# steve-the-bayesian/BOOM

Measured on AMD Instinct MI355X. Metric: Gibbs sweeps/sec (all chains), n=1e4 p=512 spike-slab, higher is better.
Workload: dtype f64; 1 GPU; BregVsSampler spike-and-slab n=1e4 p=512, 1024 chains per GPU, fp64 (BASELINE configs[1]); chains_per_gpu=1024, true_signals=16, burn_in=1000, parallelism=chains sharded, 1 GPU(s), suf_build=single device MFMA syrk

## Files before the change

boom_amd/capi.py:

```python
import ctypes as C
import os

import numpy as np

_HERE = os.path.dirname(os.path.abspath(__file__))
LIB_PATH = os.environ.get("BOOM_AMD_LIB", os.path.join(_HERE, "libboomamd.so"))

_dp = C.POINTER(C.c_double)
_u8p = C.POINTER(C.c_uint8)

SUMMARY_SCALARS = 16


class BoomAmdError(RuntimeError):

    def __init__(self, code, message):
        super().__init__(message)
        self.code = code


class BaConfig(C.Structure):
    _fields_ = [("device", C.c_int32), ("chains", C.c_int32),
                ("chain_offset", C.c_int64), ("seed", C.c_uint64),
                ("max_model_size_hint", C.c_int32), ("reserved", C.c_int32)]


_lib = None

SIGNATURES = {
    "ba_last_error": (C.c_char_p, []),
    "ba_engine_create": (C.c_int, [C.POINTER(BaConfig), C.POINTER(C.c_void_p)]),
    "ba_engine_destroy": (None, [C.c_void_p]),
    "ba_engine_info": (C.c_int, [C.c_void_p, C.POINTER(C.c_int32),
                                 C.POINTER(C.c_int32), C.POINTER(C.c_int32)]),
    "ba_build_suf_from_xy": (C.c_int, [C.c_void_p, C.c_int64, C.c_int32, _dp, _dp]),
    "ba_build_suf_from_xy_device": (C.c_int, [C.c_void_p, C.c_int64, C.c_int32,
                                              C.c_void_p, C.c_void_p]),
    "ba_suf_block_size": (C.c_size_t, [C.c_int32]),
    "ba_suf_partial_device": (C.c_int, [C.c_void_p, C.c_int64, C.c_int32, C.c_void_p,
                                        C.c_void_p, C.c_void_p]),
    "ba_set_suf_from_block_device": (C.c_int, [C.c_void_p, C.c_int64, C.c_int32, C.c_void_p]),
    "ba_upload_regression_suf": (C.c_int, [C.c_void_p, C.c_int32, _dp, _dp,
                                           C.c_double, C.c_double, C.c_double, _dp]),
    "ba_get_regression_suf": (C.c_int, [C.c_void_p, _dp, _dp, _dp, _dp, _dp, _dp]),
    "ba_set_slab": (C.c_int, [C.c_void_p, _dp, _dp]),
    "ba_set_spike": (C.c_int, [C.c_void_p, _dp, C.c_int64]),
    "ba_set_sigma_prior": (C.c_int, [C.c_void_p, C.c_double, C.c_double, C.c_double]),
    "ba_set_priors_ctor1": (C.c_int, [C.c_void_p, C.c_double, C.c_double,
                                      C.c_double, C.c_int32]),
    "ba_set_priors_ctor2": (C.c_int, [C.c_void_p, C.c_double, C.c_double,
                                      C.c_double, C.c_double, C.c_double, C.c_int32]),
    "ba_get_priors": (C.c_int, [C.c_void_p, _dp, _dp, _dp, _dp, _dp]),
    "ba_set_options": (C.c_int, [C.c_void_p, C.c_int32, C.c_double, C.c_int32, C.c_int32]),
    "ba_set_tuning": (C.c_int, [C.c_void_p, C.c_int32, C.c_int32, C.c_int32]),
    "ba_set_rebuild_policy": (C.c_int, [C.c_void_p, C.c_int32]),
    "ba_set_lookahead": (C.c_int, [C.c_void_p, C.c_int32]),
    "ba_draw_next": (C.c_int, [C.c_void_p]),
    "ba_set_state": (C.c_int, [C.c_void_p, C.c_int64, _u8p, _dp, C.c_double]),
    "ba_get_state": (C.c_int, [C.c_void_p, C.c_int64, _u8p, _dp, _dp]),
    "ba_get_states": (C.c_int, [C.c_void_p, _u8p, _dp, _dp]),
    "ba_logpri": (C.c_int, [C.c_void_p, C.c_int64, _dp]),
    "ba_seed": (C.c_int, [C.c_void_p, C.c_uint64]),
    "ba_sweep": (C.c_int, [C.c_void_p, C.c_int32]),
    "ba_sync": (C.c_int, [C.c_void_p]),
    "ba_log_model_prob": (C.c_int, [C.c_void_p, C.c_int32, _u8p, _dp]),
    "ba_set_sigsq": (C.c_int, [C.c_void_p, C.c_int64, C.c_double]),
    "ba_sss_set_slab": (C.c_int, [C.c_void_p, _dp, _dp, C.c_int32, C.c_int32]),
    "ba_sss_sweep": (C.c_int, [C.c_void_p, C.c_int32]),
    "ba_adaptive_set_options": (C.c_int, [C.c_void_p, C.c_int32, C.c_double, C.c_double]),
    "ba_adaptive_sweep": (C.c_int, [C.c_void_p, C.c_int32]),
    "ba_adaptive_get_rates": (C.c_int, [C.c_void_p, C.c_int64, _dp, _dp,
                                        C.POINTER(C.c_uint64)]),
    "ba_reset_summaries": (C.c_int, [C.c_void_p]),
    "ba_get_summaries": (C.c_int, [C.c_void_p, _dp, _dp, _dp, _dp]),
    "ba_summaries_device": (C.c_int, [C.c_void_p, C.c_void_p]),
    "ba_enable_traces": (C.c_int, [C.c_void_p, C.c_int32]),
    "ba_get_traces": (C.c_int, [C.c_void_p, C.c_int32, _dp, _dp, _dp]),
    "ba_enable_draws": (C.c_int, [C.c_void_p, C.c_int32]),
    "ba_get_draws": (C.c_int, [C.c_void_p, C.c_int64, C.c_int32, _u8p, _dp, _dp]),
    "ba_predict": (C.c_int, [C.c_void_p, C.c_int32, C.c_int32, C.c_int32, _dp, _dp]),
    "ba_get_coefficient_traces": (C.c_int, [C.c_void_p, C.c_int32, C.c_int32,
                                            C.POINTER(C.c_int32), _dp]),
    "ba_stream": (C.c_void_p, [C.c_void_p]),
    "ba_kernel_classes": (C.c_int32, []),
    "ba_kernel_class_name": (C.c_char_p, [C.c_int32]),
    "ba_set_kernel_timing": (C.c_int, [C.c_void_p, C.c_int32]),
    "ba_get_kernel_times": (C.c_int, [C.c_void_p, _dp, C.POINTER(C.c_int64), C.c_int32]),
    "ba_group_last_error": (C.c_char_p, []),
# ... 238 lines not shown

    def set_priors_ctor1(self, prior_nobs, expected_rsq, expected_model_size,
                         first_term_is_intercept=True):
        self._check(self.lib.ba_set_priors_ctor1(self._h, prior_nobs, expected_rsq,
                                                 expected_model_size,
                                                 int(first_term_is_intercept)))

    def set_priors_ctor2(self, prior_sigma_nobs, prior_sigma_guess, prior_beta_nobs,
                         diagonal_shrinkage, prior_inclusion_probability,
                         force_intercept=True):
        self._check(self.lib.ba_set_priors_ctor2(
            self._h, prior_sigma_nobs, prior_sigma_guess, prior_beta_nobs,
            diagonal_shrinkage, prior_inclusion_probability, int(force_intercept)))

    def get_priors(self):
        p = self.p
        b, om, pi = np.zeros(p), np.zeros(p * p), np.zeros(p)
        df, ss = C.c_double(), C.c_double()
        self._check(self.lib.ba_get_priors(self._h, _p(b), _p(om), _p(pi),
                                           C.byref(df), C.byref(ss)))
        return dict(b=b, ominv=om.reshape(p, p).T.copy(), pi=pi, df=df.value, ss=ss.value)

    def set_options(self, max_flips=-1, swap_threshold=0.8, draw_beta=True,
                    draw_sigma=True):
        self._check(self.lib.ba_set_options(self._h, max_flips, swap_threshold,
                                            int(draw_beta), int(draw_sigma)))

    def set_tuning(self, waves_per_chain=0, walk_policy=-1, kcap_start=0):
        self._check(self.lib.ba_set_tuning(self._h, waves_per_chain, walk_policy, kcap_start))

    def set_rebuild_policy(self, policy):
        self._check(self.lib.ba_set_rebuild_policy(self._h, int(policy)))

    def set_state(self, gamma, beta=None, sigsq=1.0, chain=-1):
        g = np.ascontiguousarray(gamma, dtype=np.uint8)
        bb = None if beta is None else _f64(beta)
        self._check(self.lib.ba_set_state(self._h, chain, _b(g), _p(bb), sigsq))

    def get_state(self, chain):
        p = self.p
        g = np.zeros(p, np.uint8)
        b = np.zeros(p)
        s = C.c_double()
        self._check(self.lib.ba_get_state(self._h, chain, _b(g), _p(b), C.byref(s)))
        return g, b, s.value

    def get_states(self):
        p, c = self.p, self.chains
        g = np.zeros((c, p), np.uint8)
        b = np.zeros((c, p))
        s = np.zeros(c)
        self._check(self.lib.ba_get_states(self._h, _b(g), _p(b), _p(s)))
        return g, b, s

    def seed(self, seed):
        self._check(self.lib.ba_seed(self._h, seed))

    def sweep(self, nsweeps=1, sync=True):
        self._check(self.lib.ba_sweep(self._h, nsweeps))
        if sync:
            self.sync()

    def sync(self):
        self._check(self.lib.ba_sync(self._h))

    def set_lookahead(self, n):
# ... 922 lines not shown
```

boom_amd/csrc/engine.hip:

```cpp
#include "engine_internal.h"

namespace boom_amd {

static thread_local std::string g_error = "";

int fail(int code, const std::string &msg) {
  g_error = msg;
  return code;
}

}

namespace {


const char *status_message(int st) {
  switch (st) {
    case CHAIN_NOT_PD:
      return "The posterior information matrix is not positive definite.  "
             "Check your data or consider adjusting your prior.";
    case CHAIN_NEGATIVE_SS:
      return "Illegal data caused negative sum of squares in "
             "Breg::set_reg_post_params.";
    case CHAIN_ILLEGAL_START:
// ... 289 lines not shown
  P.cm_idx = e->dcm_idx.ptr;
  P.cm_cor = e->dcm_cor.ptr;
  P.gamma = e->dgamma.ptr;
  P.beta = e->dbeta.ptr;
  P.sigsq = e->dsigsq.ptr;
  P.perm = e->dperm.ptr;
  P.rng_pos = e->dpos.ptr;
  P.status = e->dstatus.ptr;
  P.failures = e->dfail.ptr;
  P.todo = e->dtodo.ptr;
  P.maxk = e->dmaxk.ptr;
  P.trace_idx = e->dtrace_idx.ptr;
  P.model_scratch = e->dmodel.ptr;
  P.table_lp = e->dtab_lp.ptr;
  P.table_kind = e->dtab_kind.ptr;
  P.table_tag = e->dtab_tag.ptr;
  P.table_keep = e->table_ok ? 1 : 0;
  P.model_tag = e->dmodel_tag.ptr;
  P.model_keep = e->model_ok ? 1 : 0;
  P.suf_changed = (e->data_kind == DATA_STATE_SPACE || latent_data(e->data_kind)) ? 1 : 0;
  P.run_limit = 0;
  P.ran = nullptr;
  P.model_scratch_stride = (int64_t)ssvs_scalar_layout(64).total;
  P.big_kcap = e->big_kcap;
  P.big_model = e->dbig_model.ptr;
  P.big_model_stride = e->big_kcap > 0 ? (int64_t)ssvs_scalar_layout(e->big_kcap).total : 0;
  P.big_xs = e->dbig_xs.ptr;
  P.seed_lo = (uint32_t)e->seed;
  P.seed_hi = (uint32_t)(e->seed >> 32);
  P.stream = 0;
  P.mode = e->cur_mode;
  P.walk_policy = e->tune_walk_policy >= 0 ? e->tune_walk_policy : 1;
  P.rebuild_policy = e->tune_rebuild_policy;
  if (e->cur_mode == 1) {
    P.slab_scales = e->sss_slab_scales;
    P.stream = 3;
    P.rng_pos = e->dpos_sss.ptr;
    P.draw_sigma = 0;
    P.draw_beta = 1;
    P.cm_start = nullptr;
    P.max_flips = (e->sss_max_flips > 0) ? std::min(e->sss_max_flips, e->p) : e->p;
  }
  if (e->cur_mode == 1 && student_kind(e->data_kind) && !e->student_allow_selection)
    P.max_flips = 0;
  if (e->cur_mode == 1 && column_service(e->data_kind) && e->cols.V.count) {
    P.mode = (e->data_kind == DATA_LOGIT || e->data_kind == DATA_SS_LOGIT) ? 2 : 1;
    if (e->data_kind == DATA_MLOGIT) {
      P.mode = 3;
      P.flip_order = e->dml_order.ptr;
      P.wss = e->dml_wss.ptr;
      if (!e->mlogit_select) P.max_flips = 0;
    }
    P.V = e->cols.V.ptr;
    P.v_chain_stride = (int64_t)e->p * e->p;
    P.model_keep = 0;
    P.table_keep = 0;
    P.col_valid = e->cols.valid.ptr;
    P.col_words = e->cols.words;
    P.col_request = e->cols.wanted.ptr;
    P.v_diag = e->cols.vdiag.ptr;
  }
  if (e->cur_mode == 2) {
    P.mode = 0;
    P.stream = 4;
    P.rng_pos = e->dpos_ada.ptr;
    P.cm_start = nullptr;
// ... 864 lines not shown
  MUTATE(e);
  e->max_flips = max_flips;
  if (swap_threshold != e->swap_threshold) e->device_dirty = true;
  e->swap_threshold = swap_threshold;
  e->draw_beta = draw_beta;
  e->draw_sigma = draw_sigma;
  return BA_OK;
}

int ba_set_tuning(ba_engine *e, int32_t waves_per_chain, int32_t walk_policy,
                  int32_t kcap_start) {
  if (!e) return fail(BA_E_INVALID, "null engine");
  if (!(waves_per_chain == 0 || waves_per_chain == 1 || waves_per_chain == 2 || waves_per_chain == 4))
    return fail(BA_E_INVALID, "waves_per_chain must be 0, 1, 2 or 4");
  if (walk_policy < -1 || walk_policy > 4) return fail(BA_E_INVALID, "walk_policy must be in [-1, 4]");
  if (kcap_start < 0) return fail(BA_E_INVALID, "kcap_start must be non-negative");
  MUTATE(e);
  if (e->state_ready) {
    int rc = set_device(e);
    if (!rc) rc = ba_sync(e);
    if (rc) return rc;
  }
  e->tune_waves = waves_per_chain;
  e->tune_walk_policy = walk_policy;
  e->tune_kcap_start = kcap_start;
  e->device_dirty = true;
  return BA_OK;
}

int ba_set_rebuild_policy(ba_engine *e, int32_t policy) {
  if (!e) return fail(BA_E_INVALID, "null engine");
  if (policy != 0 && policy != 1) return fail(BA_E_INVALID, "rebuild_policy must be 0 or 1");
  e->tune_rebuild_policy = policy;
  return BA_OK;
}

int ba_set_slot_limit(ba_engine *e, int32_t uniforms) {
  if (!e) return fail(BA_E_INVALID, "null engine");
  if (uniforms < 0 || (uniforms & 1)) return fail(BA_E_INVALID, "uniforms must be even and non-negative");
  MUTATE(e);
  e->slot_limit = uniforms;
  return BA_OK;
}

int ba_set_state(ba_engine *e, int64_t chain, const uint8_t *gamma,
                 const double *beta, double sigsq) {
  ENGINE_PROLOGUE(e);
  if (e->p <= 0) return fail(BA_E_STATE, "set the regression data first");
  if (!gamma) return fail(BA_E_INVALID, "null argument");
  const int64_t C = e->cfg.chains;
  if (chain < -1 || chain >= C) return fail(BA_E_INVALID, "chain index out of range");
  if (latent_data(e->data_kind) && !student_kind(e->data_kind) && sigsq != 1.0)
    return fail(BA_E_INVALID, "the binomial samplers' latent data have unit variance: sigsq must be 1");
  if (chain < 0) la_discard(e);
  MUTATE(e);
  if (e->state_ready) {
    int rc = ba_sync(e);
    if (rc && chain >= 0) return rc;
    if (rc) {
      HIP_TRY(hipMemsetAsync(e->dstatus.ptr, 0, (size_t)C * 4, e->stream));
      HIP_TRY(hipMemsetAsync(e->dtodo.ptr, 0, (size_t)C * 4, e->stream));
    }
  }
  int rc = alloc_chain_state(e);
  if (rc) return rc;
  const size_t p = (size_t)e->p;
// ... 873 lines not shown
```

boom_amd/csrc/engine_internal.h:

```cpp
#pragma once
#include <hip/hip_runtime.h>

#include <algorithm>
#include <cmath>
#include <cstdio>
#include <cstdlib>
#include <cstring>
#include <limits>
#include <string>
#include <unordered_map>
#include <vector>

#include "../../include/boom_amd.h"
#include "kalman_params.h"
#include "ktimer.h"
#include "mlogit_params.h"
#include "probit_params.h"
#include "products.h"
#include "quantile_params.h"
#include "ss_filter_params.h"
#include "ssg_regholiday.h"
#include "ssg_spec.h"
#include "ssvs_params.h"
#include "student_params.h"
// ... 184 lines not shown
  DevBuf<int32_t> dran;
  bool table_ok = false;
  bool model_ok = false;
  int trace_stride = 0;
  DevBuf<double> dX, dy, dxtx, dxsum, dsufscal;

  int kcap = 0;
  int waves = 1;
  struct La {
    int len = 1, avail = 0, served = 0;
    struct Rows { std::vector<double> k, sig, beta; std::vector<uint16_t> idx; };
    std::unordered_map<int64_t, Rows> cache;
    bool synced = false;
    bool pipe = true;
    bool cur_piped = false;
    bool ahead = false;
    int slot = 0;
    hipEvent_t done[2] = {nullptr, nullptr};
    struct Snap {
      DevBuf<uint8_t> gamma;
      DevBuf<double> beta, sigsq, bsum, bsumsq, acc;
      DevBuf<uint16_t> perm;
      DevBuf<uint64_t> pos;
      DevBuf<int32_t> fail;
      DevBuf<uint32_t> inc;
    } snap;
  } la;
  int rec_cap = 64;
  bool big_active = false;
  int big_kcap = 0;
  DevBuf<double> dbig_model, dbig_xs;
  int tune_waves = 0, tune_walk_policy = -1, tune_kcap_start = 0;
  int tune_rebuild_policy = 0;
  int cur_mode = 0;
  int sss_slab_scales = 1;
  int sss_max_flips = -1;
  double v_scale = 1.0;
  double v_scale_want = 1.0;
  DevBuf<uint64_t> dpos_sss;
  uint64_t seed = 0;
  DevBuf<double> dada_birth, dada_death, dada_ws;
  DevBuf<uint64_t> dada_iter, dpos_ada;
  int ada_max_flips = 100;
  double ada_step = .001, ada_target = .345;

  bool ss_level_set = false, ss_initialized = false;
  int T = 0;
  DevBuf<double> dss_y, dss_X, dss_scratch;
  void *pinned = nullptr;
  size_t pinned_bytes = 0;
  uint64_t api_seq = 1, clean_seq = 0;
  int api_depth = 0;
  DevBuf<double> dss_yt, dss_Xt;
  DevBuf<uint32_t> dss_obs_mask;
  DevBuf<uint8_t> dss_obs;
  DevBuf<double> dxty_c, dyty_c, dnobs_c;
  DevBuf<double> dlev_sigsq, dlev_n, dlev_sumsq;
  DevBuf<uint64_t> dpos_level, dpos_state, dpos_forecast;
  hipStream_t stream2 = nullptr;
  hipEvent_t ev_state = nullptr, ev_prep[2] = {nullptr, nullptr};
  int ss_zbuf = 0;
  struct Pipe {
    hipStream_t stream = nullptr;
    hipEvent_t ev[4] = {}, join_ev = nullptr;
    DevBuf<int32_t> q, err;
    bool on = false;
// ... 250 lines not shown
```

boom_amd/csrc/ssvs_params.h:

```cpp
#pragma once
#include <stdint.h>

namespace boom_amd {

enum ChainStatus : int32_t {
  CHAIN_OK = 0,
  CHAIN_NOT_PD = 1,
  CHAIN_NEGATIVE_SS = 2,
  CHAIN_ILLEGAL_START = 3,
  CHAIN_RNG_BRANCH = 4,
  CHAIN_FORECAST_VARIANCE = 5,
  CHAIN_MODEL_TOO_LARGE = 6,
  CHAIN_NEED_COLUMN = 7,
  CHAIN_NEED_COLUMN_BIG = 8
};
enum { MLVS_ILLEGAL_START = 12 };

enum { SUMMARY_SCALARS = 16 };
enum {
  ACC_SWEEPS = 0,
  ACC_SIGSQ = 1,
  ACC_SIGSQ2 = 2,
  ACC_K = 3,
  ACC_ACCEPTS = 4,
// ... 76 lines not shown
  double *acc;
  double *trace_sigsq, *trace_logp, *trace_k;
  int32_t trace_stride;
  uint16_t *rec_idx;
  double *rec_beta;
  int32_t rec_cap;

  double *ada_birth, *ada_death;
  uint64_t *ada_iter;
  double ada_step, ada_target;
  int32_t ada_max_flips;
  int32_t *q_in, *q_out;
  int32_t *q_error;
  int32_t trace_row0;
  uint8_t *snap_gamma;
  double *snap_beta, *snap_sigsq, *snap_bsum, *snap_bsumsq, *snap_acc;
  uint16_t *snap_perm;
  uint64_t *snap_pos;
  int32_t *snap_fail;
  uint32_t *snap_inc;
  int32_t adaptive;
  double *ada_ws;

  int32_t big_kcap;
  double *big_model;
  int64_t big_model_stride;
  double *big_xs;
  const double *xty_planes;
  int32_t xty_nplanes;
  int64_t xty_plane_stride;
  const uint16_t *flip_order;
  const double *wss;
  int32_t rebuild_policy;
};

struct SsvsLds {
  uint32_t Lv, La, rdv, rda, w, bg, ctrl, park, g, perm0, perm1, oth, last, pred, gam, gam0, nbr, total;
};

static inline __host__ __device__ SsvsLds ssvs_lds_layout(int p, int kcap) {
  SsvsLds L;
  const uint32_t nb = (uint32_t)kcap / 8;
  const uint32_t fac = nb * (nb + 1) / 2 * 64 * 8;
  const uint32_t pv = ((((uint32_t)p + 1u) * 2) + 15u) & ~15u;
  uint32_t o = 0;
  L.Lv = o;    o += fac;
  L.La = o;    o += fac;
  L.rdv = o;   o += (uint32_t)kcap * 8;
  L.rda = o;   o += (uint32_t)kcap * 8;
  L.w = o;     o += (uint32_t)kcap * 8;
  L.bg = o;    o += (uint32_t)kcap * 8;
  L.ctrl = o;  o += 512;
  L.park = o;  o += 4 * 512;
  L.g = o;     o += (((uint32_t)kcap * 2) + 15u) & ~15u;
  L.perm0 = o; o += pv;
  L.perm1 = o; o += pv;
  L.oth = o;   o += pv;
  L.last = o;  o += 2 * pv;
  L.pred = o;  o += pv;
  L.gam = o;   o += ((uint32_t)p + 15u) & ~15u;
  L.gam0 = o;  o += ((uint32_t)p + 15u) & ~15u;
  L.nbr = o;   o += ((uint32_t)p + 15u) & ~15u;
  L.total = o;
  return L;
}

// ... 82 lines not shown
```

boom_amd/csrc/ssvs_sweep_body.h:

```cpp
#pragma once
#include "ssvs_device.h"

namespace boom_amd {

template <int NB, int W, int WPE, bool MLVS = false>
__device__ __forceinline__ void ssvs_sweep_body(SsvsParams P, int nsweeps, const int chain,
                                                unsigned char *smem) {
  constexpr bool SHUFFLE_MASKED = NB >= 6 && W > 1;
  P.V += (size_t)chain * (size_t)P.v_chain_stride;
  if (P.col_valid) {
    P.col_valid += (size_t)chain * (size_t)P.col_words;
    P.v_diag += (size_t)chain * (size_t)P.p;
  }
  int tid_ = threadIdx.x;
  BA_OPAQUE_V(tid_);
  int lane = tid_ & (WAVE - 1);
  const int wave = tid_ >> 6;
  const int p = P.p;
#ifdef BA_PSTAMPS
  long long pst[8];
  pst[0] = (long long)__builtin_readcyclecounter();
#endif
  constexpr int FOLD_Z = 16;
  const bool fold = (W == 1) && P.xty_planes != nullptr;
// ... 185 lines not shown
    if (j < p) {
      ch.gam[j] = (uint8_t)inc;
      ch.perm[j] = g_perm[j];
      ch.nbr[j] = (uint8_t)((P.cm_start != nullptr) && (P.cm_start[j + 1] > P.cm_start[j]));
    }
    const unsigned long long mask = __ballot(inc != 0);
    const int slot = k + __popcll(mask & ((1ull << lane) - 1ull));
    if (inc && slot < KCAP) ch.g[slot] = (uint16_t)j;
    k += __popcll(mask);
  }
  if (k > KCAP) status = CHAIN_MODEL_TOO_LARGE;
  ch.k = k;
  wave_sync();
  bool aborted = false;
  int need_col = -1;
  int kmax = k;
  int trace_at = (P.trace_row0 >= 0) ? P.trace_row0 : (P.trace_idx ? P.trace_idx[chain] : 0);

  uint64_t pos = uni((uint64_t)P.rng_pos[chain]);
  int failures = uni((int)P.failures[chain]);
  double sigsq = uni((double)P.sigsq[chain]);
  double beta_m = 0.0;
  int gprev = 0, kprev = 0;
  bool beta_valid = false;

  lds_f64 *sum_b = to_lds<double>(smem + lay.park + 512);
  lds_f64 *sum_b2 = to_lds<double>(smem + lay.park + 1024);
  AS_LDS int *sum_n = to_lds<int>(smem + lay.park + 1536);
  AS_LDS int *sum_g = to_lds<int>(smem + lay.park + 1792);
  sum_b[lane] = 0.0; sum_b2[lane] = 0.0; sum_n[lane] = 0; sum_g[lane] = -1;
  if (lane < 13) ctl[CT_ACC + lane] = (lane == ACC_MIN_MARGIN) ? BA_INF : 0.0;
  if (W == 2 && lane == 0) ((AS_LDS uint64_t *)(ctl + CT_NEXT))[0] = ~0ull;
  wave_sync();
#define ACC_ADD(slot, x) do { if (lane == 0) ctl[CT_ACC + (slot)] += (double)(x); } while (0)
#define ACC_MIN(x) do { if (lane == 0) ctl[CT_ACC + ACC_MIN_MARGIN] = fmin(ctl[CT_ACC + ACC_MIN_MARGIN], (x)); } while (0)
  int done = 0;

  const int nflips = P.max_flips;
  STAMP_DECL;
  StampCtx sx;
  sx.last = (long long)__builtin_readcyclecounter();
  for (int i = 0; i < 8; ++i) sx.ph[i] = 0.0;

  Model M;
  M.bad = 0; M.pd = true; M.logp = 0; M.lp = 0; M.ldv = 0; M.lda = 0; M.Q = 0; M.c = 0; M.SS = 0;
  Pending pe;
  pe.kind = EV_INIT; pe.f1 = pe.f2 = -1; pe.lu = 0; pe.lfw = pe.lrev = 0; pe.check_legal = false;
  enum { PH_BEGIN, PH_FLIPS, PH_SWAP, PH_TAIL, PH_JOIN, PH_COMMIT };
  int phase = PH_BEGIN, sweep = 0, i0 = 0;
  bool model_checked = false;
  int perm_sel = 0;
  bool use_table = false;
  int cur = 0, other_var = -1;
  bool other_ok = false, table_valid_other = false;
  const int model_tag_in = P.model_keep ? P.model_tag[chain] : 0;
  const bool model_kept = (model_tag_in & 0xff) == KCAP && status == CHAIN_OK;
  if (model_kept) cur = (model_tag_in >> 8) & 1;
  bind_slot(ch, P, chain, cur);
  bool table_valid = P.table_keep && model_kept && P.table_tag[chain] == model_tag_in;
  int fill_j = 0;
  bool spec = false;
  bool have_dr = false;
  int after_join = PH_COMMIT, spec_status = CHAIN_OK;
  bool commit_pending = false, gam0_fresh = false;
  lds_f64 *park = to_lds<double>(smem + lay.park);
  int stops_prev = table_valid ? 0 : (1 << 20), stops_now = 0;
  uint64_t flip_pos = 0, pos0 = pos;
  WinRng rng;
  rng.init(key, lane, pos);

  PSTAMP(3);
  if (model_kept) {
    {
      const SsvsScalarLayout S = ssvs_scalar_layout(KCAP);
      const double *sc = ch.sc_store + S.scal;
      const double s0 = sc[0], s1 = sc[1], s2 = sc[2], s3 = sc[3], s4 = sc[4], s5 = sc[5], s6 = sc[6], s7 = sc[7];
      restore_model<NB>(ch);
      M.logp = s0; M.lp = s1; M.ldv = s2; M.lda = s3;
      M.Q = s4; M.c = s5; M.SS = s6; M.pd = s7 != 0.0;
      unsigned long long u = (unsigned long long)ch.sc_store;
      asm volatile("s_dcache_inv\n\ts_waitcnt lgkmcnt(0)" : "+s"(u) : : "memory");
      ch.sc = (c_f64 *)u;
    }
    if (P.suf_changed) {
      refactor<true, MLVS>(P, ch, M, sx);
      if (M.bad) status = M.bad;
      else publish_model<NB>(ch, M);
    }
    if (lane == 0) {
      ctl[CT_LOGP] = M.logp; ctl[CT_LP] = M.lp; ctl[CT_LDV] = M.ldv;
      ctl[CT_LDA] = M.lda; ctl[CT_Q] = M.Q; ctl[CT_C] = M.c;
    }
    wave_sync();
    pe.kind = EV_NONE;
  }

  PSTAMP(4);
  while (status == CHAIN_OK) {
#ifdef BA_ROUND_KERNEL
    if constexpr ((W > 1 && !(NB == 4 && W == 2)) || (W == 1 && NB >= 4) || (MLVS && NB == 2)) {
#else
    constexpr bool PLAIN_211 = NB == 2 && W == 1;
    if constexpr ((W > 1 && !(NB == 4 && W == 2)) || (W == 1 && NB >= 4) || (MLVS && NB == 2) || PLAIN_211) {
#endif
      asm volatile("" : "+v"(lane));
      ch.lane = lane;
    }
    XCOUNT(sx, 6, 1);
    if (pe.kind != EV_NONE && !spec) {
      MSTAMP(sx, 7);
      XSTAMP(sx, 1);
      if (pe.kind == EV_FORCE && pe.f2 < 0 && other_ok && pe.f1 == other_var) {
        gam0_fresh = false;
        apply_flip(ch, pe.f1);
        cur ^= 1;
        bind_slot(ch, P, chain, cur);
        restore_model<NB>(ch);
        {
          const SsvsScalarLayout S = ssvs_scalar_layout(KCAP);
          const double *sc = ch.sc_store + S.scal;
          M.logp = sc[0]; M.lp = sc[1]; M.ldv = sc[2]; M.lda = sc[3];
          M.Q = sc[4]; M.c = sc[5]; M.SS = sc[6]; M.pd = sc[7] != 0.0;
          unsigned long long u = (unsigned long long)ch.sc_store;
          asm volatile("s_dcache_inv\n\ts_waitcnt lgkmcnt(0)" : "+s"(u) : : "memory");
          ch.sc = (c_f64 *)u;
        }
        if (lane == 0) {
          ctl[CT_LOGP] = M.logp; ctl[CT_LP] = M.lp; ctl[CT_LDV] = M.ldv;
          ctl[CT_LDA] = M.lda; ctl[CT_Q] = M.Q; ctl[CT_C] = M.c;
        }
        wave_sync();
        {
          const bool t = table_valid;
          table_valid = table_valid_other;
          table_valid_other = t;
        }
        ACC_ADD(ACC_ACCEPTS, 1);
#ifndef BA_STAMPS
        ACC_ADD(ACC_SLOT_HITS, 1);
#endif
// ... 132 lines not shown
            ctl[CT_ROLL + 0] = sigsq;
            ctl[CT_ROLL + 1] = (double)failures;
            ctl[CT_ROLL + 2] = beta_valid ? 1.0 : 0.0;
            ctl[CT_ROLL + 3] = 0.0;
          }
        }
        if (W > 1 && use_table && table_valid && model_checked && p > 1 && P.walk_policy != 3 && P.mode != 2 && !MLVS) {
          wave_sync();
          if (lane == 0) {
            ctl[CT_CMD] = (double)CMD_SHUFFLE_DECIDE;
            ctl[CT_I0] = 0.0;
            ctl[CT_NFLIPS] = (double)nflips;
            ctl[CT_PERMSEL] = (double)perm_sel;
            ctl[CT_CUR] = (double)cur;
            ((AS_LDS uint64_t *)(ctl + CT_POS))[0] = pos;
          }
          __syncthreads();
          fork_shuffle_targets<W>(key, pos, p, 0, lane, ch.oth);
          {
            lds_u16 *tmp = ch.perm;
            ch.perm = ch.perm_alt;
            ch.perm_alt = tmp;
            perm_sel ^= 1;
          }
          flip_pos = pos + (uint64_t)(p - 1);
          pos = flip_pos + (uint64_t)nflips;
          TSTAMP(sx, 2);
          XSTAMP(sx, 7);
          spec = true;
          spec_status = CHAIN_OK;
          i0 = 0;
          phase = commit_pending ? PH_COMMIT : PH_SWAP;
          STAMP(1);
          continue;
        }
        if constexpr (MLVS) {
          wave_sync();
          flip_pos = pos;
          pos = flip_pos + (uint64_t)nflips;
          if (!(M.logp > -BA_INF && M.logp < BA_INF)) { status = MLVS_ILLEGAL_START; aborted = true; }
        } else {
        if (W > 1) {
          if (lane == 0) {
            ctl[CT_CMD] = (double)CMD_UNIF;
            ((AS_LDS uint64_t *)(ctl + CT_POS))[0] = pos;
          }
          __syncthreads();
        }
        if (p > 1) shuffle_targets(key, pos, p, threadIdx.x, WAVE * W, ch.oth, P.mode == 2);
        if (W > 1) __syncthreads(); else wave_sync();
        STAMP(0);
        if (P.mode == 2) {
          if (lane == 0 && p > 1) {
            for (int i = 0; i < p; ++i) {
              const int j = ch.oth[i];
              const uint16_t a = ch.perm[i];
              ch.perm[i] = ch.perm[j];
              ch.perm[j] = a;
            }
          }
          wave_sync();
        } else if (p > 1) { parallel_shuffle<SHUFFLE_MASKED>(ch, sx); perm_sel ^= 1; }
        flip_pos = pos + (uint64_t)(P.mode == 2 ? p : (p > 0 ? p - 1 : 0));
        pos = flip_pos + (uint64_t)nflips;
        STAMP(1);
        if (!model_checked) {
          model_checked = true;
          if (!(M.logp > -BA_INF && M.logp < BA_INF)) {
            for (int j = 0; j < p; ++j) {
              const double pj = P.pi[j];
              const bool inc = ch.gam[j];
              if ((pj <= 0.0 && inc) || (pj >= 1.0 && !inc)) {
                if (!inc && ch.k >= KCAP) { status = CHAIN_MODEL_TOO_LARGE; aborted = true; break; }
                if (!inc && column_missing(P, j)) { status = CHAIN_NEED_COLUMN; need_col = j; aborted = true; break; }
                apply_flip(ch, j);
              }
            }
            pe.kind = EV_INIT;
            pe.check_legal = true;
          }
        }
        }
      }
      i0 = 0;
      phase = PH_FLIPS;
      XSTAMP(sx, 5);
      continue;
    }

    if (phase == PH_FLIPS) {
      XSTAMP(sx, 1);
      if (nflips == 0 || i0 >= nflips) {
        phase = PH_SWAP;
        XSTAMP(sx, 2);
        continue;
      }
      if (use_table && table_valid) {
        DecideResult dr;
        if (W > 1) {
          if (!have_dr) {
          MSTAMP(sx, 7);
          if (lane == 0) {
            ctl[CT_CMD] = (double)CMD_DECIDE;
            ctl[CT_I0] = (double)i0;
            ctl[CT_NFLIPS] = (double)nflips;
            ctl[CT_PERMSEL] = (double)perm_sel;
            ctl[CT_CUR] = (double)cur;
            ((AS_LDS uint64_t *)(ctl + CT_POS))[0] = flip_pos;
          }
          __syncthreads();
          if (P.walk_policy < 3 && P.mode != 2 && !MLVS) {
            spec = true;
            spec_status = CHAIN_OK;
            if (lane == 0) ctl[CT_ROLL + 3] = 1.0;
            MCOUNT(sx, 5, 1);
#ifndef BA_STAMPS
            ACC_ADD(ACC_REFORKS, 1);
#endif
            phase = commit_pending ? PH_COMMIT : PH_SWAP;
            XSTAMP(sx, 2);
            continue;
          }
          XSTAMP(sx, 2);
          __syncthreads();
          MSTAMP(sx, 0);
          XSTAMP(sx, 7);
          }
          have_dr = false;
          const lds_f64 *sl = ctl + CT_SLOT0 + CT_SLOT_STRIDE * 1;
// ... 102 lines not shown
      const int jf = uni((int)sl[SL_J]);
      const int kind = uni((int)sl[SL_KIND]);
      const int nprop = spos + 1 - i0;
      ACC_ADD(ACC_PROPOSALS, nprop);
      MCOUNT(sx, 4, stops_now == 0);
      ++stops_now;
      if (kind == STOP_BAD) {
        status = CHAIN_NEGATIVE_SS;
        break;
      }
      if (!ch.gam[jf] && ch.k >= KCAP) {
        status = CHAIN_MODEL_TOO_LARGE;
        aborted = true;
        break;
      }
      if (!ch.gam[jf] && column_missing(P, jf)) {
        status = CHAIN_NEED_COLUMN;
        need_col = jf;
        aborted = true;
        break;
      }
      pe.f1 = jf;
      if (kind == STOP_ACCEPT) {
        pe.kind = EV_FORCE;
      } else {
        pe.kind = EV_TRY_GE;
        pe.lu = uni((double)sl[SL_LOGU]);
      }
      i0 += nprop;
      XSTAMP(sx, 3);
      continue;
    }

    if (phase == PH_SWAP) {
      TSTAMP(sx, 7);
      XSTAMP(sx, 1);
      rng.set_pos(pos);
      if (nflips > 0) propose_swap(P, ch, rng, pe, &status);
      pos = rng.get_pos();
      phase = PH_TAIL;
      if (spec && (pe.kind != EV_NONE || status != CHAIN_OK)) {
        spec_status = status;
        status = CHAIN_OK;
        after_join = PH_TAIL;
        phase = PH_JOIN;
      }
      STAMP(4);
      TSTAMP(sx, 3);
      XSTAMP(sx, 7);
      continue;
    }

    if (phase == PH_JOIN) {
      MSTAMP(sx, 7);
      XSTAMP(sx, 1);
      __syncthreads();
      MSTAMP(sx, 1);
      XSTAMP(sx, 7);
      spec = false;
      i0 = uni((int)ctl[CT_I0]);
      const lds_f64 *sl = ctl + CT_SLOT0 + CT_SLOT_STRIDE * 1;
      if ((int)sl[SL_F] < 0) {
        ACC_MIN(sl[SL_MARGIN]);
        ACC_ADD(ACC_PROPOSALS, nflips - i0);
        status = spec_status;
        phase = after_join;
        if (after_join == PH_COMMIT && status == CHAIN_OK) {
          commit_pending = true;
          phase = PH_BEGIN;
        }
      } else {
        pos = flip_pos + (uint64_t)nflips;
        beta_m = park[lane];
        sigsq = ctl[CT_ROLL + 0];
        failures = (int)ctl[CT_ROLL + 1];
        beta_valid = ctl[CT_ROLL + 2] != 0.0;
        pe.kind = EV_NONE; pe.f1 = pe.f2 = -1; pe.lfw = pe.lrev = 0.0; pe.check_legal = false;
        have_dr = true;
        phase = PH_FLIPS;
        MCOUNT(sx, 6, ctl[CT_ROLL + 3]);
#ifndef BA_STAMPS
        ACC_ADD(ACC_REFORK_ROLLBACKS, ctl[CT_ROLL + 3]);
#endif
      }
      STAMP(3);
      XSTAMP(sx, 0);
      continue;
    }

    if (phase == PH_COMMIT) {
      TSTAMP(sx, 7);
      XSTAMP(sx, 1);
      k = ch.k;
      gprev = (lane < k) ? (int)ch.g[lane] : 0;
      kprev = k;
      kmax = k > kmax ? k : kmax;
      {
        const int gnow = (lane < k) ? gprev : -1;
        const int gold = sum_g[lane];
        if (__any(gnow != gold)) {
          const int n_old = sum_n[lane];
          if (gold >= 0 && n_old) {
            const size_t o = (size_t)chain * p + gold;
            const unsigned c0 = P.inc_count[o];
            const double b0 = P.beta_sum[o], q0 = P.beta_sumsq[o];
            P.inc_count[o] = c0 + (unsigned)n_old;
            P.beta_sum[o] = b0 + sum_b[lane];
            P.beta_sumsq[o] = q0 + sum_b2[lane];
          }
          sum_g[lane] = gnow; sum_n[lane] = 0; sum_b[lane] = 0.0; sum_b2[lane] = 0.0;
        }
        if (lane < k) {
          sum_n[lane] += 1;
          if (beta_valid) { sum_b[lane] += beta_m; sum_b2[lane] += beta_m * beta_m; }
        }
      }
      ACC_ADD(ACC_SIGSQ, sigsq);
      ACC_ADD(ACC_SIGSQ2, sigsq * sigsq);
      ACC_ADD(ACC_K, k);
      if (P.trace_sigsq && trace_at + sweep < P.trace_stride) {
        const size_t o = (size_t)chain * P.trace_stride + trace_at + sweep;
        if (lane == 0) {
          P.trace_sigsq[o] = sigsq;
          P.trace_logp[o] = M.logp;
          P.trace_k[o] = (double)k;
        }
        if (P.rec_idx && lane < k) {
          P.rec_idx[o * P.rec_cap + lane] = (uint16_t)gprev;
          P.rec_beta[o * P.rec_cap + lane] = beta_valid ? beta_m : 0.0;
        }
      }
      ++done;
      ++sweep;
      commit_pending = false;
      phase = spec ? PH_SWAP : PH_BEGIN;
      TSTAMP(sx, 0);
      XSTAMP(sx, 7);
      continue;
    }

    TSTAMP(sx, 7);
    XSTAMP(sx, 1);
    k = ch.k;
    rng.set_pos(pos);
    if (P.draw_sigma) {
      int bad = 0;
      const double DF = (k == 0) ? ch.DF : ((ch.DF - P.prior_df) + P.prior_df);
      const double SS = (k == 0) ? ch.ss0q : ((M.SS - P.prior_ss) + P.prior_ss);
      sigsq = uni(d_draw_variance(rng, DF, SS, P.sigma_max, &bad));
      if (bad) {
        if (!spec) { status = CHAIN_RNG_BRANCH; break; }
        spec_status = CHAIN_RNG_BRANCH; after_join = PH_COMMIT; phase = PH_JOIN;
        continue;
      }
    }
    pos = uni(rng.get_pos());
    STAMP(5);
    TSTAMP(sx, 4);
    if (P.draw_beta && k > 0) {
      if (!M.pd) {
        ++failures;
        if (!spec) { status = CHAIN_NOT_PD; break; }
        spec_status = CHAIN_NOT_PD; after_join = PH_COMMIT; phase = PH_JOIN;
        continue;
      }
      failures = 0;
      const double z = draw_normals(rng, k);
      pos = uni(rng.get_pos());
      TSTAMP(sx, 5);
      const double sigma = P.mode ? 1.0 : sqrt(sigsq);
      double y = (lane < k) ? ch.w[lane] + sigma * z : 0.0;
      const double rdm = (lane < k) ? ch.rdv[lane] : 0.0;
#pragma nounroll
      for (int ib = (k - 1) >> 3; ib >= 0; --ib) {
        double lr[8];
        const int base = bidx(ib * 8, lane < ib * 8 + 8 ? lane : 0);
#pragma unroll
        for (int t = 0; t < 8; ++t) lr[t] = ch.Lv[base + t * 8];
#pragma unroll
        for (int t = 7; t >= 0; --t) {
          const int i = ib * 8 + t;
          if (i < k) {
            const double xi = bcast_u(y * rdm, i);
            if (lane == i) y = xi;
            else if (lane < i) y -= lr[t] * xi;
          }
        }
      }
      beta_m = y;
      beta_valid = true;
      TSTAMP(sx, 6);
    } else if (P.draw_beta) {
      beta_valid = true;
    }
    STAMP(6);
    XSTAMP(sx, 7);
    after_join = PH_COMMIT;
    if (W == 2 && !MLVS && spec && lane == 0) ((AS_LDS uint64_t *)(ctl + CT_NEXT))[0] = pos;
    phase = spec ? PH_JOIN : PH_COMMIT;
  }

  PSTAMP(5);
  if (W > 1) {
    if (lane == 0) ctl[CT_CMD] = (double)CMD_EXIT;
    __syncthreads();
  }

  wave_sync();
#ifndef BA_STAMPS
  double *acc_row = P.acc + (size_t)chain * ACC_COUNT;
  const double acc_old = (lane < 13) ? acc_row[lane] : 0.0;
#endif
  if (sum_g[lane] >= 0 && sum_n[lane]) {
    const size_t o = (size_t)chain * p + sum_g[lane];
    P.inc_count[o] += (unsigned)sum_n[lane];
    P.beta_sum[o] += sum_b[lane];
    P.beta_sumsq[o] += sum_b2[lane];
  }
  wave_sync();
  {
    const lds_u8 *gsrc = aborted ? ch.gam0 : ch.gam;
    const lds_u16 *psrc = (aborted && p > 1) ? ch.perm_alt : ch.perm;
    for (int j = lane; j < p; j += WAVE) {
      g_gamma[j] = gsrc[j];
      g_perm[j] = psrc[j];
    }
    if (aborted) pos = pos0;
  }
  if (beta_valid) {
    double *g_beta = P.beta + (size_t)chain * p;
    for (int j = lane; j < p; j += WAVE) g_beta[j] = 0.0;
    wave_sync();
// ... 57 lines not shown
```

include/boom_amd.h:

```cpp
#ifndef BOOM_AMD_H
#define BOOM_AMD_H

#include <stddef.h>
#include <stdint.h>

#ifdef __cplusplus
extern "C" {
#endif

enum {
  BA_OK = 0,
  BA_E_INVALID = -1,
  BA_E_HIP = -2,
  BA_E_NOT_PD = -3,
  BA_E_NEGATIVE_SS = -4,
  BA_E_ILLEGAL_START = -5,
  BA_E_RNG_BRANCH = -6,
  BA_E_FORECAST_VARIANCE = -7,
  BA_E_MODEL_TOO_LARGE = -8,
  BA_E_STATE = -9
};

typedef struct ba_engine ba_engine;

// ... 22 lines not shown
                          const void *X_device, const void *y_device,
                          void *block_device);
int ba_set_suf_from_block_device(ba_engine *e, int64_t n_total, int32_t p,
                                 const void *block_device);
int ba_upload_regression_suf(ba_engine *e, int32_t p, const double *xtx,
                             const double *xty, double yty, double n,
                             double ybar, const double *xbar);
int ba_get_regression_suf(ba_engine *e, double *xtx, double *xty, double *yty,
                          double *n, double *ybar, double *xbar);

int ba_set_slab(ba_engine *e, const double *prior_mean,
                const double *unscaled_prior_precision);
int ba_set_spike(ba_engine *e, const double *prior_inclusion_probabilities,
                 int64_t max_model_size);
int ba_set_sigma_prior(ba_engine *e, double prior_df, double sigma_guess,
                       double sigma_upper_limit);
int ba_set_priors_ctor1(ba_engine *e, double prior_nobs, double expected_rsq,
                        double expected_model_size,
                        int32_t first_term_is_intercept);
int ba_set_priors_ctor2(ba_engine *e, double prior_sigma_nobs,
                        double prior_sigma_guess, double prior_beta_nobs,
                        double diagonal_shrinkage,
                        double prior_inclusion_probability,
                        int32_t force_intercept);
int ba_get_priors(ba_engine *e, double *prior_mean, double *ominv, double *pi,
                  double *prior_df, double *prior_ss);

int ba_set_options(ba_engine *e, int32_t max_flips, double swap_threshold,
                   int32_t draw_beta, int32_t draw_sigma);

int ba_set_tuning(ba_engine *e, int32_t waves_per_chain, int32_t walk_policy,
                  int32_t kcap_start);
int ba_set_rebuild_policy(ba_engine *e, int32_t policy);
int ba_set_slot_limit(ba_engine *e, int32_t uniforms);

int ba_set_state(ba_engine *e, int64_t chain, const uint8_t *gamma,
                 const double *beta, double sigsq);
int ba_get_state(ba_engine *e, int64_t chain, uint8_t *gamma, double *beta,
                 double *sigsq);
int ba_get_states(ba_engine *e, uint8_t *gamma, double *beta, double *sigsq);
int ba_logpri(ba_engine *e, int64_t chain, double *out);
int ba_seed(ba_engine *e, uint64_t seed);

int ba_sweep(ba_engine *e, int32_t nsweeps);
int ba_sync(ba_engine *e);
int ba_set_lookahead(ba_engine *e, int32_t lookahead);
int ba_draw_next(ba_engine *e);
int ba_log_model_prob(ba_engine *e, int32_t ngamma, const uint8_t *gammas,
                      double *out);

int ba_set_sigsq(ba_engine *e, int64_t chain, double sigsq);
int ba_sss_set_slab(ba_engine *e, const double *mu, const double *precision,
                    int32_t precision_scales_with_sigsq, int32_t max_flips);
int ba_sss_sweep(ba_engine *e, int32_t nsweeps);

int ba_adaptive_set_options(ba_engine *e, int32_t max_flips, double step_size,
                            double target_acceptance_rate);
int ba_adaptive_sweep(ba_engine *e, int32_t nsweeps);
int ba_adaptive_get_rates(ba_engine *e, int64_t chain, double *birth_rates,
                          double *death_rates, uint64_t *iteration_count);

int ba_probit_set_data(ba_engine *e, int64_t n, int32_t p, const double *X,
                       const double *y, const double *ntrials, int32_t clt_threshold);
int ba_probit_sweep(ba_engine *e, int32_t nsweeps);

int ba_logit_set_data(ba_engine *e, int64_t n, int32_t p, const double *X,
// ... 210 lines not shown
```

Measured before the change: 68.33 million sweeps/s.

## Let sweep phases fall through instead of looping back through the dispatcher

Restructures the per-chain phase state machine so BEGIN→FLIPS→SWAP→TAIL→COMMIT can fall through directly, skipping a trip back to the top of the loop when the wave is uniform. The commit step moves into an inlined lambda and is run straight after a speculative join for two-wave chains, with no extra pass through the loop. This is meant to cut loop-dispatch overhead and branch or sync cost per sweep. It adds a runtime phase_policy knob (default 0 enables fallthrough) and compiler barriers on the accumulator macros. In exchange it adds code size and register pressure.

```diff
diff --git a/boom_amd/capi.py b/boom_amd/capi.py
--- a/boom_amd/capi.py
+++ b/boom_amd/capi.py
@@ -54,6 +54,7 @@
     "ba_set_options": (C.c_int, [C.c_void_p, C.c_int32, C.c_double, C.c_int32, C.c_int32]),
     "ba_set_tuning": (C.c_int, [C.c_void_p, C.c_int32, C.c_int32, C.c_int32]),
     "ba_set_rebuild_policy": (C.c_int, [C.c_void_p, C.c_int32]),
+    "ba_set_phase_policy": (C.c_int, [C.c_void_p, C.c_int32]),
     "ba_set_lookahead": (C.c_int, [C.c_void_p, C.c_int32]),
     "ba_draw_next": (C.c_int, [C.c_void_p]),
     "ba_set_state": (C.c_int, [C.c_void_p, C.c_int64, _u8p, _dp, C.c_double]),
@@ -358,6 +359,9 @@
     def set_rebuild_policy(self, policy):
         self._check(self.lib.ba_set_rebuild_policy(self._h, int(policy)))
 
+    def set_phase_policy(self, policy):
+        self._check(self.lib.ba_set_phase_policy(self._h, int(policy)))
+
     def set_state(self, gamma, beta=None, sigsq=1.0, chain=-1):
         g = np.ascontiguousarray(gamma, dtype=np.uint8)
         bb = None if beta is None else _f64(beta)
diff --git a/boom_amd/csrc/engine.hip b/boom_amd/csrc/engine.hip
--- a/boom_amd/csrc/engine.hip
+++ b/boom_amd/csrc/engine.hip
@@ -345,6 +345,7 @@
   P.mode = e->cur_mode;
   P.walk_policy = e->tune_walk_policy >= 0 ? e->tune_walk_policy : 1;
   P.rebuild_policy = e->tune_rebuild_policy;
+  P.phase_policy = e->tune_phase_policy;
   if (e->cur_mode == 1) {
     P.slab_scales = e->sss_slab_scales;
     P.stream = 3;
@@ -1275,6 +1276,13 @@
   if (!e) return fail(BA_E_INVALID, "null engine");
   if (policy != 0 && policy != 1) return fail(BA_E_INVALID, "rebuild_policy must be 0 or 1");
   e->tune_rebuild_policy = policy;
+  return BA_OK;
+}
+
+int ba_set_phase_policy(ba_engine *e, int32_t policy) {
+  if (!e) return fail(BA_E_INVALID, "null engine");
+  if (policy < 0 || policy > 2) return fail(BA_E_INVALID, "phase_policy must be 0, 1 or 2");
+  e->tune_phase_policy = policy;
   return BA_OK;
 }
 
diff --git a/boom_amd/csrc/engine_internal.h b/boom_amd/csrc/engine_internal.h
--- a/boom_amd/csrc/engine_internal.h
+++ b/boom_amd/csrc/engine_internal.h
@@ -240,6 +240,7 @@
   DevBuf<double> dbig_model, dbig_xs;
   int tune_waves = 0, tune_walk_policy = -1, tune_kcap_start = 0;
   int tune_rebuild_policy = 0;
+  int tune_phase_policy = 0;
   int cur_mode = 0;
   int sss_slab_scales = 1;
   int sss_max_flips = -1;
diff --git a/boom_amd/csrc/ssvs_params.h b/boom_amd/csrc/ssvs_params.h
--- a/boom_amd/csrc/ssvs_params.h
+++ b/boom_amd/csrc/ssvs_params.h
@@ -132,6 +132,7 @@
   const uint16_t *flip_order;
   const double *wss;
   int32_t rebuild_policy;
+  int32_t phase_policy;
 };
 
 struct SsvsLds {
diff --git a/boom_amd/csrc/ssvs_sweep_body.h b/boom_amd/csrc/ssvs_sweep_body.h
--- a/boom_amd/csrc/ssvs_sweep_body.h
+++ b/boom_amd/csrc/ssvs_sweep_body.h
@@ -241,8 +241,8 @@
   if (lane < 13) ctl[CT_ACC + lane] = (lane == ACC_MIN_MARGIN) ? BA_INF : 0.0;
   if (W == 2 && lane == 0) ((AS_LDS uint64_t *)(ctl + CT_NEXT))[0] = ~0ull;
   wave_sync();
-#define ACC_ADD(slot, x) do { if (lane == 0) ctl[CT_ACC + (slot)] += (double)(x); } while (0)
-#define ACC_MIN(x) do { if (lane == 0) ctl[CT_ACC + ACC_MIN_MARGIN] = fmin(ctl[CT_ACC + ACC_MIN_MARGIN], (x)); } while (0)
+#define ACC_ADD(slot, x) do { if (lane == 0) ctl[CT_ACC + (slot)] += (double)(x); asm volatile(""); } while (0)
+#define ACC_MIN(x) do { if (lane == 0) ctl[CT_ACC + ACC_MIN_MARGIN] = fmin(ctl[CT_ACC + ACC_MIN_MARGIN], (x)); asm volatile(""); } while (0)
   int done = 0;
 
   const int nflips = P.max_flips;
@@ -304,17 +304,78 @@
     pe.kind = EV_NONE;
   }
 
+#ifdef BA_ROUND_KERNEL
+  constexpr bool PLAIN_211 = false;
+#else
+  constexpr bool PLAIN_211 = NB == 2 && W == 1;
+#endif
+  constexpr bool OPAQUE_LANE = (W > 1 && !(NB == 4 && W == 2)) || (W == 1 && NB >= 4) || (MLVS && NB == 2) || PLAIN_211;
+#define LANE_OPAQUE() do { if constexpr (OPAQUE_LANE) { asm volatile("" : "+v"(lane)); ch.lane = lane; } } while (0)
+#ifdef BA_ROUND_KERNEL
+  constexpr bool ROUND = true;
+#else
+  constexpr bool ROUND = false;
+#endif
+  constexpr bool ENTRY_OPAQUE = ROUND && NB == 4;
+#define LANE_OPAQUE_ENTRY() do { if constexpr (ENTRY_OPAQUE) LANE_OPAQUE(); } while (0)
+
+  constexpr bool FALL_CT = !(PLAIN_211 || W == 4 || (NB == 8 && W == 2) || (ROUND && NB != 4));
+  const bool fall = FALL_CT && P.phase_policy != 1;
+  const bool join_commit = FALL_CT && W == 2 && !MLVS && P.phase_policy == 0 && fork_targets_solo<W>(p) && P.walk_policy < 3;
+  auto commit_sweep = [&]() __attribute__((always_inline)) {
+    TSTAMP(sx, 7);
+    XSTAMP(sx, 1);
+    k = ch.k;
+    gprev = (lane < k) ? (int)ch.g[lane] : 0;
+    kprev = k;
+    kmax = k > kmax ? k : kmax;
+    {
+      const int gnow = (lane < k) ? gprev : -1;
+      const int gold = sum_g[lane];
+      if (__any(gnow != gold)) {
+        const int n_old = sum_n[lane];
+        if (gold >= 0 && n_old) {
+          const size_t o = (size_t)chain * p + gold;
+          const unsigned c0 = P.inc_count[o];
+          const double b0 = P.beta_sum[o], q0 = P.beta_sumsq[o];
+          P.inc_count[o] = c0 + (unsigned)n_old;
+          P.beta_sum[o] = b0 + sum_b[lane];
+          P.beta_sumsq[o] = q0 + sum_b2[lane];
+        }
+        sum_g[lane] = gnow; sum_n[lane] = 0; sum_b[lane] = 0.0; sum_b2[lane] = 0.0;
+      }
+      if (lane < k) {
+        sum_n[lane] += 1;
+        if (beta_valid) { sum_b[lane] += beta_m; sum_b2[lane] += beta_m * beta_m; }
+      }
+    }
+    ACC_ADD(ACC_SIGSQ, sigsq);
+    ACC_ADD(ACC_SIGSQ2, sigsq * sigsq);
+    ACC_ADD(ACC_K, k);
+    if (P.trace_sigsq && trace_at + sweep < P.trace_stride) {
+      const size_t o = (size_t)chain * P.trace_stride + trace_at + sweep;
+      if (lane == 0) {
+        P.trace_sigsq[o] = sigsq;
+        P.trace_logp[o] = M.logp;
+        P.trace_k[o] = (double)k;
+      }
+      if (P.rec_idx && lane < k) {
+        P.rec_idx[o * P.rec_cap + lane] = (uint16_t)gprev;
+        P.rec_beta[o * P.rec_cap + lane] = beta_valid ? beta_m : 0.0;
+      }
+    }
+    ++done;
+    ++sweep;
+    commit_pending = false;
+    phase = spec ? PH_SWAP : PH_BEGIN;
+    TSTAMP(sx, 0);
+    XSTAMP(sx, 7);
+  };
+
+
   PSTAMP(4);
   while (status == CHAIN_OK) {
-#ifdef BA_ROUND_KERNEL
-    if constexpr ((W > 1 && !(NB == 4 && W == 2)) || (W == 1 && NB >= 4) || (MLVS && NB == 2)) {
-#else
-    constexpr bool PLAIN_211 = NB == 2 && W == 1;
-    if constexpr ((W > 1 && !(NB == 4 && W == 2)) || (W == 1 && NB >= 4) || (MLVS && NB == 2) || PLAIN_211) {
-#endif
-      asm volatile("" : "+v"(lane));
-      ch.lane = lane;
-    }
+    LANE_OPAQUE();
     XCOUNT(sx, 6, 1);
     if (pe.kind != EV_NONE && !spec) {
       MSTAMP(sx, 7);
@@ -513,8 +574,9 @@
           i0 = 0;
           phase = commit_pending ? PH_COMMIT : PH_SWAP;
           STAMP(1);
-          continue;
-        }
+          if (!fall) continue;
+        }
+        if (!spec) {
         if constexpr (MLVS) {
           wave_sync();
           flip_pos = pos;
@@ -562,20 +624,26 @@
           }
         }
         }
-      }
-      i0 = 0;
-      phase = PH_FLIPS;
-      XSTAMP(sx, 5);
-      continue;
+        }
+      }
+      if (!spec) {
+        i0 = 0;
+        phase = PH_FLIPS;
+        XSTAMP(sx, 5);
+        if (!fall || uni(status) != CHAIN_OK || uni((int)pe.kind) != EV_NONE) continue;
+      }
+    }
+
+    if (phase == PH_FLIPS && (nflips == 0 || i0 >= nflips)) {
+      XSTAMP(sx, 1);
+      phase = PH_SWAP;
+      XSTAMP(sx, 2);
+      if (!fall) continue;
     }
 
     if (phase == PH_FLIPS) {
+      LANE_OPAQUE_ENTRY();
       XSTAMP(sx, 1);
-      if (nflips == 0 || i0 >= nflips) {
-        phase = PH_SWAP;
-        XSTAMP(sx, 2);
-        continue;
-      }
       if (use_table && table_valid) {
         DecideResult dr;
         if (W > 1) {
@@ -744,7 +812,13 @@
       continue;
     }
 
+    if (phase == PH_COMMIT) {
+      commit_sweep();
+      if (!(fall && spec)) continue;
+    }
+
     if (phase == PH_SWAP) {
+      LANE_OPAQUE_ENTRY();
       TSTAMP(sx, 7);
       XSTAMP(sx, 1);
       rng.set_pos(pos);
@@ -760,10 +834,75 @@
       STAMP(4);
       TSTAMP(sx, 3);
       XSTAMP(sx, 7);
-      continue;
+      if (!fall || uni(phase) != PH_TAIL || uni(status) != CHAIN_OK || uni((int)pe.kind) != EV_NONE) continue;
+    }
+
+    if (phase == PH_TAIL) {
+      LANE_OPAQUE_ENTRY();
+      TSTAMP(sx, 7);
+      XSTAMP(sx, 1);
+      k = ch.k;
+      rng.set_pos(pos);
+      if (P.draw_sigma) {
+        int bad = 0;
+        const double DF = (k == 0) ? ch.DF : ((ch.DF - P.prior_df) + P.prior_df);
+        const double SS = (k == 0) ? ch.ss0q : ((M.SS - P.prior_ss) + P.prior_ss);
+        sigsq = uni(d_draw_variance(rng, DF, SS, P.sigma_max, &bad));
+        if (bad) {
+          if (!spec) { status = CHAIN_RNG_BRANCH; break; }
+          spec_status = CHAIN_RNG_BRANCH; after_join = PH_COMMIT; phase = PH_JOIN;
+          continue;
+        }
+      }
+      pos = uni(rng.get_pos());
+      STAMP(5);
+      TSTAMP(sx, 4);
+      if (P.draw_beta && k > 0) {
+        if (!M.pd) {
+          ++failures;
+          if (!spec) { status = CHAIN_NOT_PD; break; }
+          spec_status = CHAIN_NOT_PD; after_join = PH_COMMIT; phase = PH_JOIN;
+          continue;
+        }
+        failures = 0;
+        const double z = draw_normals(rng, k);
+        pos = uni(rng.get_pos());
+        TSTAMP(sx, 5);
+        const double sigma = P.mode ? 1.0 : sqrt(sigsq);
+        double y = (lane < k) ? ch.w[lane] + sigma * z : 0.0;
+        const double rdm = (lane < k) ? ch.rdv[lane] : 0.0;
+#pragma nounroll
+        for (int ib = (k - 1) >> 3; ib >= 0; --ib) {
+          double lr[8];
+          const int base = bidx(ib * 8, lane < ib * 8 + 8 ? lane : 0);
+#pragma unroll
+          for (int t = 0; t < 8; ++t) lr[t] = ch.Lv[base + t * 8];
+#pragma unroll
+          for (int t = 7; t >= 0; --t) {
+            const int i = ib * 8 + t;
+            if (i < k) {
+              const double xi = bcast_u(y * rdm, i);
+              if (lane == i) y = xi;
+              else if (lane < i) y -= lr[t] * xi;
+            }
+          }
+        }
+        beta_m = y;
+        beta_valid = true;
+        TSTAMP(sx, 6);
+      } else if (P.draw_beta) {
+        beta_valid = true;
+      }
+      STAMP(6);
+      XSTAMP(sx, 7);
+      after_join = PH_COMMIT;
+      if (W == 2 && !MLVS && spec && lane == 0) ((AS_LDS uint64_t *)(ctl + CT_NEXT))[0] = pos;
+      phase = spec ? PH_JOIN : PH_COMMIT;
+      if (!(fall && spec)) continue;
     }
 
     if (phase == PH_JOIN) {
+      LANE_OPAQUE_ENTRY();
       MSTAMP(sx, 7);
       XSTAMP(sx, 1);
       __syncthreads();
@@ -772,13 +911,15 @@
       spec = false;
       i0 = uni((int)ctl[CT_I0]);
       const lds_f64 *sl = ctl + CT_SLOT0 + CT_SLOT_STRIDE * 1;
+      bool commit_now = false;
       if ((int)sl[SL_F] < 0) {
         ACC_MIN(sl[SL_MARGIN]);
         ACC_ADD(ACC_PROPOSALS, nflips - i0);
         status = spec_status;
         phase = after_join;
         if (after_join == PH_COMMIT && status == CHAIN_OK) {
-          commit_pending = true;
+          commit_now = join_commit;
+          commit_pending = !join_commit;
           phase = PH_BEGIN;
         }
       } else {
@@ -797,119 +938,8 @@
       }
       STAMP(3);
       XSTAMP(sx, 0);
-      continue;
-    }
-
-    if (phase == PH_COMMIT) {
-      TSTAMP(sx, 7);
-      XSTAMP(sx, 1);
-      k = ch.k;
-      gprev = (lane < k) ? (int)ch.g[lane] : 0;
-      kprev = k;
-      kmax = k > kmax ? k : kmax;
-      {
-        const int gnow = (lane < k) ? gprev : -1;
-        const int gold = sum_g[lane];
-        if (__any(gnow != gold)) {
-          const int n_old = sum_n[lane];
-          if (gold >= 0 && n_old) {
-            const size_t o = (size_t)chain * p + gold;
-            const unsigned c0 = P.inc_count[o];
-            const double b0 = P.beta_sum[o], q0 = P.beta_sumsq[o];
-            P.inc_count[o] = c0 + (unsigned)n_old;
-            P.beta_sum[o] = b0 + sum_b[lane];
-            P.beta_sumsq[o] = q0 + sum_b2[lane];
-          }
-          sum_g[lane] = gnow; sum_n[lane] = 0; sum_b[lane] = 0.0; sum_b2[lane] = 0.0;
-        }
-        if (lane < k) {
-          sum_n[lane] += 1;
-          if (beta_valid) { sum_b[lane] += beta_m; sum_b2[lane] += beta_m * beta_m; }
-        }
-      }
-      ACC_ADD(ACC_SIGSQ, sigsq);
-      ACC_ADD(ACC_SIGSQ2, sigsq * sigsq);
-      ACC_ADD(ACC_K, k);
-      if (P.trace_sigsq && trace_at + sweep < P.trace_stride) {
-        const size_t o = (size_t)chain * P.trace_stride + trace_at + sweep;
-        if (lane == 0) {
-          P.trace_sigsq[o] = sigsq;
-          P.trace_logp[o] = M.logp;
-          P.trace_k[o] = (double)k;
-        }
-        if (P.rec_idx && lane < k) {
-          P.rec_idx[o * P.rec_cap + lane] = (uint16_t)gprev;
-          P.rec_beta[o * P.rec_cap + lane] = beta_valid ? beta_m : 0.0;
-        }
-      }
-      ++done;
-      ++sweep;
-      commit_pending = false;
-      phase = spec ? PH_SWAP : PH_BEGIN;
-      TSTAMP(sx, 0);
-      XSTAMP(sx, 7);
-      continue;
-    }
-
-    TSTAMP(sx, 7);
-    XSTAMP(sx, 1);
-    k = ch.k;
-    rng.set_pos(pos);
-    if (P.draw_sigma) {
-      int bad = 0;
-      const double DF = (k == 0) ? ch.DF : ((ch.DF - P.prior_df) + P.prior_df);
-      const double SS = (k == 0) ? ch.ss0q : ((M.SS - P.prior_ss) + P.prior_ss);
-      sigsq = uni(d_draw_variance(rng, DF, SS, P.sigma_max, &bad));
-      if (bad) {
-        if (!spec) { status = CHAIN_RNG_BRANCH; break; }
-        spec_status = CHAIN_RNG_BRANCH; after_join = PH_COMMIT; phase = PH_JOIN;
-        continue;
-      }
-    }
-    pos = uni(rng.get_pos());
-    STAMP(5);
-    TSTAMP(sx, 4);
-    if (P.draw_beta && k > 0) {
-      if (!M.pd) {
-        ++failures;
-        if (!spec) { status = CHAIN_NOT_PD; break; }
-        spec_status = CHAIN_NOT_PD; after_join = PH_COMMIT; phase = PH_JOIN;
-        continue;
-      }
-      failures = 0;
-      const double z = draw_normals(rng, k);
-      pos = uni(rng.get_pos());
-      TSTAMP(sx, 5);
-      const double sigma = P.mode ? 1.0 : sqrt(sigsq);
-      double y = (lane < k) ? ch.w[lane] + sigma * z : 0.0;
-      const double rdm = (lane < k) ? ch.rdv[lane] : 0.0;
-#pragma nounroll
-      for (int ib = (k - 1) >> 3; ib >= 0; --ib) {
-        double lr[8];
-        const int base = bidx(ib * 8, lane < ib * 8 + 8 ? lane : 0);
-#pragma unroll
-        for (int t = 0; t < 8; ++t) lr[t] = ch.Lv[base + t * 8];
-#pragma unroll
-        for (int t = 7; t >= 0; --t) {
-          const int i = ib * 8 + t;
-          if (i < k) {
-            const double xi = bcast_u(y * rdm, i);
-            if (lane == i) y = xi;
-            else if (lane < i) y -= lr[t] * xi;
-          }
-        }
-      }
-      beta_m = y;
-      beta_valid = true;
-      TSTAMP(sx, 6);
-    } else if (P.draw_beta) {
-      beta_valid = true;
-    }
-    STAMP(6);
-    XSTAMP(sx, 7);
-    after_join = PH_COMMIT;
-    if (W == 2 && !MLVS && spec && lane == 0) ((AS_LDS uint64_t *)(ctl + CT_NEXT))[0] = pos;
-    phase = spec ? PH_JOIN : PH_COMMIT;
+      if (commit_now) commit_sweep();
+    }
   }
 
   PSTAMP(5);
diff --git a/include/boom_amd.h b/include/boom_amd.h
--- a/include/boom_amd.h
+++ b/include/boom_amd.h
@@ -78,6 +78,7 @@
 int ba_set_tuning(ba_engine *e, int32_t waves_per_chain, int32_t walk_policy,
                   int32_t kcap_start);
 int ba_set_rebuild_policy(ba_engine *e, int32_t policy);
+int ba_set_phase_policy(ba_engine *e, int32_t policy);
 int ba_set_slot_limit(ba_engine *e, int32_t uniforms);
 
 int ba_set_state(ba_engine *e, int64_t chain, const uint8_t *gamma,
```

After: 68.80 million sweeps/s, median of 6. Within noise of the previous version (+0.7%).
